# Kira7dn/Low_Level_Feature_Extraction

Hardware: AMD Instinct MI355X
Metric: images/sec, 1080p batch, full colors+shapes+shadows pipeline @1/2/4/8 MI355X (higher is better)
Workload: dtype u8

## Files before the change

low_level_feature_extraction_amd/csrc/kmeans.hip:

```cpp
#include "kmeans_common.h"

#include <mutex>
#include <type_traits>

namespace llfe {
namespace {

#ifndef LLFE_KM_CELL_MIN
#define LLFE_KM_CELL_MIN 8192
#endif
constexpr int kCellMinCubes = LLFE_KM_CELL_MIN;
#ifndef LLFE_KM_SPLIT
#define LLFE_KM_SPLIT 0
#endif
#ifndef LLFE_KM_LLOYD_QUEUE
#define LLFE_KM_LLOYD_QUEUE 0
#endif
#ifndef LLFE_KM_SUPS
#define LLFE_KM_SUPS 1
#endif
#ifndef LLFE_KM_WIDE
#define LLFE_KM_WIDE 0
#endif
#ifndef LLFE_KM_THREADS
// ... 151 lines not shown
    union {
        struct {
            unsigned long long psum[3][kParts];
            unsigned long long pD[kParts];
            unsigned long long wchunk[3][KW];
            int marg[kMaxK * kMaxK + 6 * kMaxK];
            int margc[kMaxK * kMaxK + 6 * kMaxK];
            int margs[kMaxK * kMaxK + 6 * kMaxK];
        } ppw;
        uint32_t pend[KW][kPend];
    };
    unsigned long long pex[3];
    unsigned long long S[3];
    uint32_t pbase[kParts + 1];
    uint32_t kbeg[kParts];
    uint32_t kfirst, klast;
    int pj[3];
    int icc[kMaxK][3];
    unsigned long long sel_pts;
    uint32_t stage[KW][kStage + 64];
    float thrL[3][kMaxK * kMaxK];
    int cq[KW][256];
    unsigned long long qtot;
};

static_assert(sizeof(KmSmem) * (1024 / KT) <= 160 * 1024, "KmSmem must leave room for 1024 / KT workgroups per CU");
static_assert(offsetof(KmSmem, accB) == sizeof(((KmSmem *)nullptr)->accA) &&
                  3 * KW * kSelSteps * sizeof(uint32_t) <= 2 * sizeof(((KmSmem *)nullptr)->accA),
              "selection step sums overflow the Lloyd accumulators (KT too small)");
static_assert(KW > 4 || sizeof(((KmSmem *)nullptr)->pend) <= sizeof(((KmSmem *)nullptr)->ppw),
              "pending-cube lists overflow the k-means++ state they alias");
static_assert(kPend >= 63 + 64 && (kPend & (kPend - 1)) == 0, "pending-cube list too small");

__device__ __forceinline__ Cent load_centres(const float (*c)[3]) {
    Cent r;
#pragma unroll
    for (int k = 0; k < kMaxK; k++) {
        r.x[k] = uni(c[k][0]);
        r.y[k] = uni(c[k][1]);
        r.z[k] = uni(c[k][2]);
    }
    return r;
}

__device__ __forceinline__ int moved_label(const KmSmem &sm, int i, int l) {
    for (int m = 0; m < sm.n_moved; m++)
        if (sm.moved_idx[m] == i) l = sm.moved_lbl[m];
    return l;
}

__device__ __forceinline__ int d2i(int x, int y, int z, int cx, int cy, int cz) {
    const int a = x - cx, b = y - cy, c = z - cz;
    return __mul24(a, a) + __mul24(b, b) + __mul24(c, c);
}

// ... 108 lines not shown
                      gz = (int)__builtin_rintf(az * (2.f * sc));
            p = kBisBand - ((int)__builtin_rintf(f0 * sc) + 3 * (gx + gy + gz));
            s1 = gz;
            s2 = gy - 3 * gz;
            s3 = gx - 3 * (gy + gz);
        }
        const uint32_t mlo = (uint32_t)e.mask, mhi = (uint32_t)(e.mask >> 32);
        const uint4 sg = bisector_signs(p, s1, s2, s3);
        const MaskMoments a = mask_moments(mlo & sg.x, mhi & sg.y), b = mask_moments(mlo & sg.z, mhi & sg.w);
        atomicAdd(&sm.accA[k][tid], (unsigned long long)(a.n * (uint32_t)ox + a.sx) |
                                        ((unsigned long long)(a.n * (uint32_t)oy + a.sy) << 32));
        atomicAdd(&sm.accB[k][tid], (unsigned long long)(a.n * (uint32_t)oz + a.sz) | ((unsigned long long)a.n << 32));
        atomicAdd(&sm.accA[jc][tid], (unsigned long long)(b.n * (uint32_t)ox + b.sx) |
                                         ((unsigned long long)(b.n * (uint32_t)oy + b.sy) << 32));
        atomicAdd(&sm.accB[jc][tid], (unsigned long long)(b.n * (uint32_t)oz + b.sz) | ((unsigned long long)b.n << 32));
        r.x = mlo & ~(sg.x | sg.z);
        r.y = mhi & ~(sg.y | sg.w);
        r.z = cube_origin_key(e.id);
        r.w = a.n + b.n;
    }
    return r;
}

__device__ __noinline__ uint2 gain_signs(int q, int s1, int s2, int s3) {
    uint32_t w[2] = {0u, 0u};
#pragma unroll
    for (int bit = 63; bit >= 0; bit--) {
        const int h = bit >> 5;
        w[h] = __builtin_amdgcn_alignbit(w[h], (uint32_t)q, 31);
        if (bit > 0) q += (bit & 15) == 0 ? s3 : ((bit & 3) == 0 ? s2 : s1);
    }
    return make_uint2(w[0], w[1]);
}

struct PPSplit {
    uint32_t und;
    int f[3];
    u16x2 krb;
    int ky;
};

__device__ __forceinline__ uint32_t lane_off_rel(int fill) { return (uint32_t)(__lane_id() - fill); }

constexpr int CPF = 1;
struct CubeRing {
    CubeEnt r[CPF];
    __device__ __forceinline__ void init(const CubeEnt *t, int cb, int cend, int lane) {
#pragma unroll
        for (int q = 0; q < CPF; q++) {
            r[q].mask = 0;
            r[q].id = 0;
            r[q].sums = 0;
            if (cb + q * 64 + lane < cend) r[q] = t[cb + q * 64 + lane];
        }
    }
    __device__ __forceinline__ CubeEnt next(const CubeEnt *t, int ci, int cend) {
        const CubeEnt e = r[0];
#pragma unroll
        for (int q = 0; q + 1 < CPF; q++) r[q] = r[q + 1];
        if (ci + CPF * 64 < cend) r[CPF - 1] = t[ci + CPF * 64];
        return e;
    }
// ... 46 lines not shown
        const uint32_t y = __shfl_up(x, off), hy = __shfl_up(hx, off);
        if (lane >= off) x += y, hx += hy;
    }
    const uint32_t pb = x - v, kb = hx - hv;
    sm.pbase[lane] = pb;
    sm.kbeg[lane] = kb;
    if (lane == 63) sm.pbase[kParts] = x;
    const unsigned long long ne = __ballot(v != 0);
    const int p0 = ne ? (int)__builtin_ctzll(ne) : 0, pl = ne ? 63 - (int)__builtin_clzll(ne) : 0;
    const uint32_t kf = __shfl(kb, p0), kl = __shfl(kb, pl) + __shfl(v, pl) - 1;
    if (lane == 0) {
        sm.kfirst = kf;
        sm.klast = kl;
    }
    const unsigned long long le = __ballot(pb <= idx);
    const int P = le ? 63 - (int)__builtin_clzll(le) : 0;
    return __shfl(kb, P) + (idx - __shfl(pb, P));
}

__device__ void pp_cubes(KmSmem &sm, const uint32_t *__restrict__ pts, int N, int K, uint64_t &rng,
                         const CubeEnt *__restrict__ ctab, int C, const CellEnt *__restrict__ ltab, int L,
                         const SupEnt *__restrict__ stab, int S, const uint32_t *__restrict__ part_uq, const uint32_t *__restrict__ hist,
                         const uint64_t *__restrict__ mom, unsigned long long &bytes, uint32_t &pp_pts, uint32_t &pp_sel, uint64_t &t_sel,
                         uint32_t &pp_split_cubes, uint32_t &pp_split_pts) {
    const int tid = threadIdx.x, lane = tid & 63, wid = tid >> 6;
    const uint32_t c0 = cvrng_next(rng) % (uint32_t)N;
    if (wid == 0) {
        const uint32_t a0 = key_layout(sm, part_uq, hist, c0);
        if (lane == 0) {
            const uint32_t q0 = pts[a0];
            sm.icc[0][0] = unpack_r(q0);
            sm.icc[0][1] = unpack_g(q0);
            sm.icc[0][2] = unpack_b(q0);
        }
    }
    if (tid == 0) {
        sm.fail_pts = 0;
        sm.sel_pts = 0;
    }
    if (tid >= 64 && tid < 64 + (kMaxK - 1) * 3) (&sm.icc[1][0])[tid - 64] = 0;
    unsigned long long mq[kPartMoments];
    if (wid == 1) {
#pragma unroll
        for (int q = 0; q < kPartMoments; q++) mq[q] = mom[q * kParts + lane];
    }
    __syncthreads();
    if (wid == 1) {
        const unsigned long long cx = (unsigned long long)sm.icc[0][0], cy = (unsigned long long)sm.icc[0][1],
// ... 332 lines not shown
    #pragma unroll
                for (int m = 1; m < kMaxK; m++) {
                    if (m >= KK) break;
                    Dk = k == m ? Dc[m] : Dk;
                    ky = k == m ? chg2[m] : ky;
                    krb = k == m ? chrb[m] : krb;
                }
                bool owned = true;
    #pragma unroll
                for (int m = 0; m < kMaxK; m++) {
                    if (m >= KK) break;
                    if (m != k) owned = owned & (Dc[m] - Dk - MK[m * kMaxK + k] >= 0);
                }
                const int sk = sdot(krb, ky);
                bool dec = true;
                uint32_t vv[3], und = 0u;
    #pragma unroll
                for (int j = 0; j < 3; j++) {
                    const int f = T2[j] - odot(trb[j], tg2[j]) - Dk;
                    const bool A = f - NAx[j * kMaxK + k] >= 0;
                    const bool B = f + NBx[j * kMaxK + k] <= 0;
                    dec = dec & (A | (owned & B));
                    vv[j] = A ? 0u : (uint32_t)(sdot(trb[j], tg2[j]) - sk - __mul24(n, f));
                    if (sp) {
                        sp->f[j] = f;
                        und |= (uint32_t)(owned & !A & !B) << j;
                    }
                }
                if (sp) {
                    sp->und = und;
                    sp->krb = krb;
                    sp->ky = ky;
                }
                v0 = vv[0];
                v1 = vv[1];
                v2 = vv[2];
                fail = !dec;
            };
            auto cube_vals = [&](const CubeEnt &e, uint32_t &v0, uint32_t &v1, uint32_t &v2, bool &fail,
                                 PPSplit *sp) __attribute__((always_inline)) {
                const CubeGeo g = cube_geo(e);
                box_vals(g.ox, g.oy, g.oz, g.n, g.sx, g.sy, g.sz, g.s2, Mkk, NA, NB, 3, 3, 3, v0, v1, v2, fail, sp);
            };
            auto split_owned = [&](const CubeEnt &e, const PPSplit &sp, uint32_t v0, uint32_t v1, uint32_t v2,
                                   bool &fail) __attribute__((always_inline)) {
                if (kPPSplitMin > 64) return;
                const bool so = fail && sp.und != 0u;
                const unsigned long long sb = __ballot(so);
                if (__popcll(sb) < kPPSplitMin) return;
                spl_cubes += (uint32_t)__popcll(sb);
                uint32_t und = 0u;
                if (so) {
                    und = sp.und;
                    acc0 += (und & 1u) ? 0u : v0;
                    acc1 += (und & 2u) ? 0u : v1;
                    acc2 += (und & 4u) ? 0u : v2;
                    spl_pts += e.sums & 127u;
                    fail = false;
                }
                const uint32_t mlo = (uint32_t)e.mask, mhi = (uint32_t)(e.mask >> 32);
                const uint32_t tw0 = __builtin_bit_cast(uint32_t, trb[0]), tw1 = __builtin_bit_cast(uint32_t, trb[1]),
                               tw2 = __builtin_bit_cast(uint32_t, trb[2]);
                const uint32_t kw = __builtin_bit_cast(uint32_t, sp.krb);
                while (__ballot(und != 0u)) {
                    if (und) {
                        const uint32_t m0 = 0u - (und & 1u), m1 = ~m0 & (0u - ((und >> 1) & 1u)), m2 = ~(m0 | m1);
                        und &= und - 1u;
                        const int f = (int)(((uint32_t)sp.f[0] & m0) | ((uint32_t)sp.f[1] & m1) | ((uint32_t)sp.f[2] & m2));
                        const uint32_t tw = (tw0 & m0) | (tw1 & m1) | (tw2 & m2);
                        const int tg = (int)(((uint32_t)tg2[0] & m0) | ((uint32_t)tg2[1] & m1) | ((uint32_t)tg2[2] & m2));
                        const int gx = (int)(tw >> 16) - (int)(kw >> 16), gy = tg - sp.ky,
                                  gz = (int)(tw & 0xFFFFu) - (int)(kw & 0xFFFFu);
                        const uint2 pos = gain_signs(f - 3 * (gx + gy + gz), gz, gy - 3 * gz, gx - 3 * (gy + gz));
                        const MaskMoments a = mask_moments(mlo & pos.x, mhi & pos.y);
                        const uint32_t g = (uint32_t)(__mul24(gx, (int)a.sx) + __mul24(gy, (int)a.sy) + __mul24(gz, (int)a.sz) -
                                                      __mul24((int)a.n, f));
                        acc0 += g & m0;
                        acc1 += g & m1;
                        acc2 += g & m2;
                    }
                }
            };
            auto push_cubes = [&](unsigned long long fm, const CubeEnt &e) __attribute__((always_inline)) {
                const uint32_t okey = cube_origin_key(e.id);
                const uint32_t mlo = (uint32_t)e.mask, mhi = (uint32_t)(e.mask >> 32);
                while (fm) {
    #pragma unroll
                    for (int u = 0; u < LLFE_KM_UNROLL; u++) {
                        if (u > 0 && !fm) break;
                        const int src = __builtin_ctzll(fm);
                        fm = clear_bit(fm, src);
                        const unsigned long long m =
                            ((unsigned long long)(uint32_t)__builtin_amdgcn_readlane(mhi, src) << 32) |
                            (uint32_t)__builtin_amdgcn_readlane(mlo, src);
                        const uint32_t r = __builtin_amdgcn_mbcnt_hi((uint32_t)(m >> 32),
                                                                     __builtin_amdgcn_mbcnt_lo((uint32_t)m, 0u));
                        stg[lane_sel(m, ((uint32_t)head + r) & (kStage - 1), kStage + lane)] =
                            (uint32_t)__builtin_amdgcn_readlane(okey, src) | loff;
                        head += __popcll(m);
                    }
                    while (head - tail >= 64) sum_stage(64);
                }
            };
            auto next_part = [&](int Pseg) __attribute__((always_inline)) {
// ... 35 lines not shown
                        if (cf) {
    #pragma unroll
                            for (uint32_t jj = 0; jj < 4; jj++)
                                if (jj <= nc1) ql[pre + jj] = (int)(e.first + jj);
                        }
                        __builtin_amdgcn_wave_barrier();
                        for (int b = 0; b < total; b += 64) {
                            const bool cv = b + lane < total;
                            CubeEnt ce;
                            ce.mask = 0;
                            ce.id = 0;
                            ce.sums = 0;
                            if (cv) ce = ctab[ql[b + lane]];
                            uint32_t c0 = 0, c1 = 0, c2 = 0;
                            bool cfail = false;
                            PPSplit sp;
                            sp.und = 0u;
                            if (cv) cube_vals(ce, c0, c1, c2, cfail, &sp);
                            if (cv && !cfail) {
                                acc0 += c0;
                                acc1 += c1;
                                acc2 += c2;
                            }
                            split_owned(ce, sp, c0, c1, c2, cfail);
                            const unsigned long long fm = __ballot(cv && cfail);
                            if (fm) push_cubes(fm, ce);
                        }
                        __builtin_amdgcn_wave_barrier();
                    }
                };
                int run = __builtin_amdgcn_readfirstlane(grab());
                int base = run;
                int ahead = grab();
                CellEnt en{0u, 0u, 0u, 0u};
                if (base + lane < L) en = ltab[base + lane];
                while (base < L) {
                    const bool valid = base + lane < L;
                    const CellEnt e = en;
                    int nb = base + 64;
                    if (nb >= run + kRun || nb >= L) {
                        run = __builtin_amdgcn_readfirstlane(ahead);
                        nb = run;
                        if (nb < L) ahead = grab();
                    }
                    if (nb + lane < L) en = ltab[nb + lane];
                    const int P = valid ? (int)((e.id >> 10) & 63u) : kParts;
                    uint32_t v0 = 0, v1 = 0, v2 = 0;
// ... 37 lines not shown
                    const int P = valid ? (int)((e.id >> 12) & 63u) : kParts;
                    uint32_t v0 = 0, v1 = 0, v2 = 0;
                    bool fail = false;
                    if (valid) cube_vals(e, v0, v1, v2, fail, nullptr);
                    int Pseg = __shfl(P, 0);
                    for (;;) {
                        next_part(Pseg);
                        const bool mine = P == Pseg;
                        if (mine && !fail) {
                            acc0 += v0;
                            acc1 += v1;
                            acc2 += v2;
                        }
                        const unsigned long long fm = __ballot(mine && fail);
                        if (fm) push_cubes(fm, e);
                        const unsigned long long rest = __ballot(P > Pseg && P < kParts);
                        if (!rest) break;
                        Pseg = __shfl(P, (int)__builtin_ctzll(rest));
                    }
                    base = nb;
            }
            }
            if (Pcur >= 0) {
                flush_pk();
                const unsigned long long a0 = wave_sum(acc0), a1 = wave_sum(acc1), a2 = wave_sum(acc2);
                if (lane == 0) {
                    atomicAdd(&sm.ppw.psum[0][Pcur], a0);
                    atomicAdd(&sm.ppw.psum[1][Pcur], a1);
                    atomicAdd(&sm.ppw.psum[2][Pcur], a2);
                }
            }
            if (lane == 0 && fails) atomicAdd(&sm.fail_pts, fails);
            if (spl_cubes) {
                const uint32_t np = wave_sum(spl_pts);
                if (lane == 0) {
                    atomicAdd(&sm.split_cubes, (unsigned long long)spl_cubes);
                    atomicAdd(&sm.split_pts, (unsigned long long)np);
                }
            }
        };
        switch (kk) {
            case 1: sweep(std::integral_constant<int, 1>{}); break;
            case 2: sweep(std::integral_constant<int, 2>{}); break;
            case 3: sweep(std::integral_constant<int, 3>{}); break;
            default: sweep(std::integral_constant<int, kMaxK - 1>{}); break;
        }
        __syncthreads();
        if (wid == 0) {
#pragma unroll
            for (int j = 0; j < 3; j++) {
                const unsigned long long s = wave_sum(sm.ppw.psum[j][lane]);
                if (lane == 0) sm.S[j] = sum0 - s;
            }
        }
        __syncthreads();
        int best = 0;
        double bs = 1.7976931348623157e308;
        for (int j = 0; j < 3; j++)
            if ((double)sm.S[j] < bs) {
                bs = (double)sm.S[j];
                best = j;
            }
        sum0 = sm.S[best];
        if (tid < kParts) sm.ppw.pD[tid] -= sm.ppw.psum[best][tid];
        if (tid == 0) {
            sm.icc[kk][0] = best == 0 ? tx[0] : (best == 1 ? tx[1] : tx[2]);
            sm.icc[kk][1] = best == 0 ? ty[0] : (best == 1 ? ty[1] : ty[2]);
            sm.icc[kk][2] = best == 0 ? tz[0] : (best == 1 ? tz[1] : tz[2]);
        }
    }
    __syncthreads();
    if (tid < kMaxK * 3) {
        const int k = tid / 3, j = tid % 3;
        sm.cc[k][j] = k < K ? (float)sm.icc[k][j] : kFar;
    }
    if (tid == 0) {
        bytes += 16ull * (unsigned long long)C * (unsigned long long)K + 4ull * sm.sel_pts;
        pp_pts = (uint32_t)sm.fail_pts;
        pp_sel = (uint32_t)sm.sel_pts;
        pp_split_cubes = (uint32_t)sm.split_cubes;
        pp_split_pts = (uint32_t)sm.split_pts;
        sm.fail_pts = sm.split_cubes = sm.split_pts = 0;
    }
    __syncthreads();
}

#ifndef LLFE_KM_MINW
#define LLFE_KM_MINW 4
#endif

template <bool kCubes, int kPhase, bool kQueue>
__global__ __launch_bounds__(KT, LLFE_KM_MINW) void k_kmeans(const uint32_t *__restrict__ keys, long long key_stride,
                                                   const long long *__restrict__ n_unique, int n_colors,
                                                   unsigned long long seed, ImgIndex index,
                                                   const int *__restrict__ order, int n_tasks,
                                                   int *__restrict__ queue, uint32_t *__restrict__ scratch,
                                                   long long scratch_stride, KmeansAttemptOut *__restrict__ out,
                                                   const KmeansCubes cubes) {
    static_assert(kPhase == 3 || kCubes, "the plain path runs both phases in one workgroup");
    extern __shared__ __attribute__((aligned(16))) char smem_raw[];
    KmSmem &sm = *reinterpret_cast<KmSmem *>(smem_raw);
    const int tid = threadIdx.x, lane = tid & 63, wid = tid >> 6;
    int task = (int)blockIdx.x;
    if (kQueue) {
// ... 13 lines not shown
    if (tid == 0) {
        unsigned hw, xcc;
        asm volatile("s_getreg_b32 %0, hwreg(HW_REG_HW_ID)" : "=s"(hw));
        asm volatile("s_getreg_b32 %0, hwreg(HW_REG_XCC_ID)" : "=s"(xcc));
        const uint64_t t = wall_clock64();
        if (kPhase & 1) {
            o->t_start = t;
            o->hw_id = hw;
            o->xcc_id = xcc;
        }
        if (kPhase & 2) {
            o->t_lstart = t;
            o->hw_id2 = hw;
            o->xcc_id2 = xcc;
        }
    }
    if (K <= 1) {
        if (tid == 0) {
            o->compactness = 0.0;
            o->iters = 0;
            o->bytes = 0;
            o->pp_pts = 0;
            o->pp_split_cubes = o->pp_split_pts = 0;
            o->n_cubes = 0;
            o->t_sel = 0;
            o->ll_pts = 0;
            o->split_cubes = o->split_pts = 0;
            o->split_walks = o->split_partial = 0;
            o->t_sw = 0;
            o->drift_hist = 0;
            o->pad = 0;
            o->t_end = wall_clock64();
            if (kPhase == 2) {
                o->t_start = o->t_pp = o->t_lstart;
                o->hw_id = o->hw_id2;
                o->xcc_id = o->xcc_id2;
            }
        }
        goto next_task;
    }
    const uint32_t *pts = keys + (size_t)img * key_stride;
    const int M = (N + STEP - 1) / STEP;
    const int Mw = (M + KW - 1) / KW;
    const int sb = min(M, wid * Mw), se = min(M, sb + Mw);
    const int se_full = max(sb, min(se, N / STEP));
    uint32_t *ss = scratch + ((size_t)img * kAttempts + att) * (size_t)scratch_stride;
    constexpr bool use_cubes = kCubes;
    const int C = use_cubes ? cubes.n_cubes[img] : 0;
    const CubeEnt *ctab = use_cubes ? cubes.cubes + (size_t)img * cubes.cube_stride : nullptr;
    uint32_t pp_pts = 0, pp_sel = 0, pp_split_cubes = 0, pp_split_pts = 0;
    uint64_t t_sel = 0, ll_pts = 0;
    unsigned long long bytes = use_cubes ? 0ull : 4ull * (unsigned long long)N * (unsigned long long)(K + 1);
    if (tid == 0) {
        sm.fail_pts = sm.split_cubes = sm.split_pts = 0;
        sm.split_walks = sm.split_partial = 0;
    }
#define SSLOT(slot) (ss + (size_t)(slot) * (size_t)M)

    if (kPhase & 1) {
    uint64_t rng = splitmix64(seed + (unsigned long long)index.at(img));
    if (rng == 0) rng = 0xFFFFFFFFull;
    for (int q = 0, skip = att * (1 + 6 * (K - 1)); q < skip; q++) cvrng_next(rng);

    if (use_cubes) {
        pp_cubes(sm, pts, N, K, rng, ctab, C, cubes.cells + (size_t)img * cubes.cell_stride, cubes.n_cells[img],
                 cubes.sups ? cubes.sups + (size_t)img * cubes.sup_stride : nullptr, cubes.sups ? cubes.n_sups[img] : 0,
                 cubes.part_uq + (size_t)img * kParts, cubes.part_hist ? cubes.part_hist + (size_t)img * kParts : nullptr,
                 cubes.moments + (size_t)img * kPartMoments * kParts, bytes, pp_pts, pp_sel, t_sel, pp_split_cubes, pp_split_pts);
    } else {
    int cur = 0;
    {
        const uint32_t c0 = cvrng_next(rng) % (uint32_t)N;
        const P3 q0 = unpack(pts[c0]);
        if (tid == 0) {
            sm.cc[0][0] = q0.x; sm.cc[0][1] = q0.y; sm.cc[0][2] = q0.z;
        }
        const float cx = uni(q0.x), cy = uni(q0.y), cz = uni(q0.z);
        unsigned long long wt = 0;
        for (int s = sb; s < se; s++) {
            const int i0 = s * STEP + lane * 4;
            uint32_t ls = 0;
            if (s < se_full) {
                uint4 v = *(const uint4 *)(pts + i0);
                uint32_t kq[4] = {v.x, v.y, v.z, v.w};
#pragma unroll
                for (int j = 0; j < 4; j++) {
                    P3 p = unpack(kq[j]);
                    ls += (uint32_t)d2(p.x, p.y, p.z, cx, cy, cz);
                }
            } else {
                for (int j = 0; j < 4; j++)
// ... 174 lines not shown
        sum0 = S[best];
        cur = best == 0 ? sl0 : (best == 1 ? sl1 : sl2);
        __syncthreads();
        if (tid == 0) {
            sm.cc[kk][0] = tc.x[best];
            sm.cc[kk][1] = tc.y[best];
            sm.cc[kk][2] = tc.z[best];
        }
        __syncthreads();
    }

    }
    if (tid == 0) o->t_pp = wall_clock64();
    if (tid < kMaxK * 3) (&o->pp_centers[0][0])[tid] = sm.cc[tid / 3][tid % 3];
    }
    if (kPhase == 1) {
        if (tid < kMaxK * 3) (&o->centers[0][0])[(tid / 3) * 3 + tid % 3] = sm.cc[tid / 3][tid % 3];
        if (tid == 0) {
            o->qtot = sm.qtot;
            o->bytes = bytes;
            o->pp_pts = pp_pts;
            o->pp_split_cubes = pp_split_cubes;
            o->pp_split_pts = pp_split_pts;
            o->pad = (int32_t)pp_sel;
            o->t_sel = t_sel;
        }
        goto next_task;
    }
    if (kPhase == 2) {
        if (tid < kMaxK * 3) {
            const int k = tid / 3, j = tid % 3;
            sm.cc[k][j] = k < K ? o->centers[k][j] : kFar;
        }
        if (tid == 0) sm.qtot = o->qtot;
        bytes = o->bytes;
        __syncthreads();
    }
    if (tid < kMaxK * 3) {
        int k = tid / 3, j = tid % 3;
        sm.c[k][j] = k < K ? sm.cc[k][j] : kFar;
    }
    __syncthreads();

    auto thr_tables = [&](int q) {
        const int k = q / kMaxK, j = q % kMaxK;
        const float dx = fabsf(sm.c[j][0] - sm.c[k][0]), dy = fabsf(sm.c[j][1] - sm.c[k][1]),
                    dz = fabsf(sm.c[j][2] - sm.c[k][2]);
        const bool none = j == k || j >= K || k >= K;
        sm.thrL[0][q] = none ? -__builtin_inff() : 3.f * (dx + dy + dz) + 1.f;
        sm.thrL[1][q] = none ? -__builtin_inff() : 3.f * dx + 7.f * (dy + dz) + 1.f;
        sm.thrL[2][q] = none ? -__builtin_inff() : 3.f * dx + 15.f * (dy + dz) + 1.f;
    };
    if (tid == 0) sm.next_chunk = 0;
    if (use_cubes && tid < kMaxK * kMaxK) thr_tables(tid);
#pragma unroll
    for (int k = 0; k < kMaxK; k++) {
        sm.accA[k][tid] = 0;
        sm.accB[k][tid] = 0;
    }
    __syncthreads();
    int iter = 1;
    const double eps2 = 0.2 * 0.2;
    uint64_t t_sw = 0;
    uint64_t drift_hist = 0;
    for (;;) {
        const uint64_t tsw0 = wall_clock64();
        const CentP c = pack_centres(load_centres(sm.c));
        if (use_cubes) {
            const Cent cu = load_centres(sm.c);
            f2 lw_x[3], lw_y[3], lw_z[3], lc2[3];
#pragma unroll
            for (int j = 0; j < 3; j++) {
#pragma unroll
                for (int h = 0; h < 2; h++) {
                    const int m = 2 * j + h;
                    const bool used = m < K;
                    const float cx = m < kMaxK ? cu.x[m] : 0.f, cy = m < kMaxK ? cu.y[m] : 0.f,
                                cz = m < kMaxK ? cu.z[m] : 0.f;
                    const float wx = used ? -2.f * cx : 0.f, wy = used ? -2.f * cy : 0.f, wz = used ? -2.f * cz : 0.f;
                    const float c2 = used ? cx * cx + cy * cy + cz * cz : __builtin_inff();
                    if (h == 0) {
                        lw_x[j].x = wx, lw_y[j].x = wy, lw_z[j].x = wz, lc2[j].x = c2;
                    } else {
                        lw_x[j].y = wx, lw_y[j].y = wy, lw_z[j].y = wz, lc2[j].y = c2;
                    }
                }
            }
// ... 307 lines not shown
                        unsigned long long b = (unsigned long long)(kq[jj] & 255u) | (1ull << 32);
                        atomicAdd(&sm.accA[l][tid], a);
                        atomicAdd(&sm.accB[l][tid], b);
                    }
                }
#pragma unroll
                for (int d = 0; d < PF; d++) cur[d] = nxt[d];
            }
        }
        for (int s = se_full; s < se; s++) {
            const int i0 = s * STEP + lane * 4;
            for (int jj = 0; jj < 4; jj++) {
                if (i0 + jj >= N) break;
                uint32_t kq = pts[i0 + jj];
                int l = label5p(kq, c);
                atomicAdd(&sm.accA[l][tid], (unsigned long long)((kq >> 16) & 255u) |
                                                ((unsigned long long)((kq >> 8) & 255u) << 32));
                atomicAdd(&sm.accB[l][tid], (unsigned long long)(kq & 255u) | (1ull << 32));
            }
        }
        }
        __syncthreads();
        t_sw += wall_clock64() - tsw0;
        if (tid == 0) {
            if (use_cubes) {
                bytes += 16ull * (unsigned long long)C;
                ll_pts += sm.fail_pts;
                sm.fail_pts = 0;
            } else {
                bytes += 4ull * (unsigned long long)N;
            }
        }
        for (int q = tid; q < 640; q += KT) {
            constexpr int LPP = KT / 32;
            const int v = q >> 5, part = q & 31;
            const int k = v >> 2, comp = v & 3;
            unsigned long long acc = 0;
            const unsigned long long *src = comp < 2 ? sm.accA[k] : sm.accB[k];
#pragma unroll 4
            for (int j = 0; j < LPP; j++) {
                unsigned long long wv = src[part + 32 * j];
                acc += (comp & 1) ? (wv >> 32) : (wv & 0xFFFFFFFFull);
            }
            sm.red[part][v] = acc;
        }
        __syncthreads();
#pragma unroll
        for (int k = 0; k < kMaxK; k++) {
            sm.accA[k][tid] = 0;
            sm.accB[k][tid] = 0;
        }
        for (int pass = 0;; pass++) {
            if (wid == 0) {
                const int v = lane < 20 ? lane : 0, k = v >> 2, comp = v & 3;
                unsigned long long val = 0;
                bool go = true;
                if (pass == 0) {
                    if (lane < 20) {
                        for (int part = 0; part < 32; part++) val += sm.red[part][v];
                        if (comp < 3) {
                            sm.sums[k][comp] = (long long)val;
                            sm.cprev[k][comp] = sm.c[k][comp];
                        } else {
                            sm.counts[k] = (int)val;
                        }
                    }
                    go = !__ballot(lane < 20 && comp == 3 && k < K && val == 0);
                    if (lane == 0) {
                        sm.n_moved = 0;
                        sm.flag = go ? 0 : 2;
                    }
                } else {
                    val = comp < 3 ? (unsigned long long)sm.sums[k][comp] : (unsigned long long)sm.counts[k];
                }
                if (go) {
                    const int count = (int)__shfl(val, v | 3);
                    const float scale = 1.f / (float)count;
                    const float nv = (float)(long long)val * scale;
                    const double t = (double)(nv - (comp < 3 ? sm.cprev[k][comp] : 0.f));
                    const double t2 = t * t;
                    double dist = 0.0;
                    dist += __shfl(t2, 4 * k);
                    dist += __shfl(t2, 4 * k + 1);
                    dist += __shfl(t2, 4 * k + 2);
                    if (lane < 20 && comp < 3 && k < K) sm.c[k][comp] = nv;
                    double max_shift = 0.0;
#pragma unroll
                    for (int k1 = 0; k1 < kMaxK; k1++) {
                        const double dk = __shfl(dist, 4 * k1);
                        if (k1 < K) max_shift = fmax(max_shift, dk);
                    }
                    if (use_cubes) {
                        __builtin_amdgcn_wave_barrier();
                        if (lane < kMaxK * kMaxK) thr_tables(lane);
                    }
                    if (lane == 0) {
                        sm.flag = (iter + 1 == 100 || max_shift <= eps2) ? 1 : 0;
                        sm.next_chunk = 0;
                        const int bin = (max_shift >= 0.0625) + (max_shift >= 0.25) + (max_shift >= 1.0) +
                                        (max_shift >= 4.0) + (max_shift >= 16.0) + (max_shift >= 64.0) +
                                        (max_shift >= 256.0);
                        const unsigned long long sh = 8ull * (unsigned)bin;
                        if (((drift_hist >> sh) & 255ull) < 255ull) drift_hist += 1ull << sh;
                    }
                }
            }
            __syncthreads();
            if (sm.flag != 2) break;

        for (int ek = 0; ek < K; ek++) {
            if (sm.counts[ek] != 0) continue;
            int max_k = 0;
            for (int k1 = 1; k1 < K; k1++)
                if (sm.counts[max_k] < sm.counts[k1]) max_k = k1;
            const float scale = 1.f / (float)sm.counts[max_k];
            const float bx = (float)sm.sums[max_k][0] * scale, by = (float)sm.sums[max_k][1] * scale,
                        bz = (float)sm.sums[max_k][2] * scale;
            const Cent cp = load_centres(sm.cprev);
            double md = -1.0;
            int mi = -1;
            auto visit = [&](int i) {
                P3 pp = unpack(pts[i]);
                float bd;
                int l = moved_label(sm, i, label5(pp, cp, bd));
                if (l != max_k) return;
                double d = (double)d2(pp.x, pp.y, pp.z, bx, by, bz);
// ... 44 lines not shown
                    }
                if (bi >= 0) {
                    P3 pp = unpack(pts[bi]);
                    sm.counts[max_k]--;
                    sm.counts[ek]++;
                    sm.sums[max_k][0] -= (long long)pp.x;
                    sm.sums[max_k][1] -= (long long)pp.y;
                    sm.sums[max_k][2] -= (long long)pp.z;
                    sm.sums[ek][0] += (long long)pp.x;
                    sm.sums[ek][1] += (long long)pp.y;
                    sm.sums[ek][2] += (long long)pp.z;
                    sm.moved_idx[sm.n_moved] = bi;
                    sm.moved_lbl[sm.n_moved] = ek;
                    sm.n_moved++;
                }
            }
            __syncthreads();
        }
        }
        iter++;
        if (sm.flag) break;
    }

    if (tid == 0) o->t_lloyd = wall_clock64();
    if (use_cubes) {
        if (tid == 0) {
            double acc = (double)sm.qtot;
            for (int k = 0; k < K; k++) {
                double cs = 0.0, c2 = 0.0;
                for (int j = 0; j < 3; j++) {
                    const double cj = (double)sm.c[k][j];
                    cs += cj * (double)sm.sums[k][j];
                    c2 += cj * cj;
                }
                acc -= 2.0 * cs - (double)sm.counts[k] * c2;
            }
            sm.dred[0] = acc;
            for (int w = 1; w < KW; w++) sm.dred[w] = 0.0;
        }
        __syncthreads();
    } else {
        const Cent cp = load_centres(sm.cprev);
        const Cent cn = load_centres(sm.c);
        const bool moved = sm.n_moved > 0;
        double acc = 0.0;
        for (int s = sb; s < se; s++) {
            const int i0 = s * STEP + lane * 4;
// ... 9 lines not shown
                for (int k = 1; k < kMaxK; k++) {
                    cx = l == k ? cn.x[k] : cx;
                    cy = l == k ? cn.y[k] : cy;
                    cz = l == k ? cn.z[k] : cz;
                }
                acc += (double)d2(pp.x, pp.y, pp.z, cx, cy, cz);
            }
        }
        acc = wave_sum(acc);
        if (lane == 0) sm.dred[wid] = acc;
        __syncthreads();
    }
    {
        if (tid == 0) {
            double compactness = 0.0;
            for (int w = 0; w < KW; w++) compactness += sm.dred[w];
            o->compactness = compactness;
            o->iters = iter;
            o->bytes = bytes;
            if (kPhase & 1) {
                o->pp_pts = pp_pts;
                o->pp_split_cubes = pp_split_cubes;
                o->pp_split_pts = pp_split_pts;
                o->pad = (int32_t)pp_sel;
                o->t_sel = t_sel;
            }
            o->ll_pts = ll_pts;
            o->split_cubes = sm.split_cubes;
            o->split_pts = sm.split_pts;
            o->split_walks = sm.split_walks;
            o->split_partial = sm.split_partial;
            o->t_sw = t_sw;
            o->n_cubes = (uint32_t)C;
            o->drift_hist = drift_hist;
            o->t_end = wall_clock64();
            for (int k = 0; k < kMaxK; k++) {
                for (int j = 0; j < 3; j++) o->centers[k][j] = k < K ? sm.c[k][j] : 0.f;
                o->counts[k] = k < K ? sm.counts[k] : 0;
            }
        }
    }
    }
    next_task:
    if (!kQueue) break;
    __syncthreads();
    if (tid == 0) sm.task = atomicAdd(queue, 1);
    __syncthreads();
    task = sm.task;
    __syncthreads();
    }
}


constexpr int OT = 1024;
constexpr int OMAX = 4096;
__global__ __launch_bounds__(OT) void k_kmeans_order(const long long *__restrict__ n_unique, int n,
                                                     int *__restrict__ order) {
// ... 157 lines not shown
```

low_level_feature_extraction_amd/csrc/kmeans_big.hip:

```cpp
#include "kmeans_common.h"

namespace llfe {
namespace {

using namespace km;

constexpr int BT = 512;
constexpr int BW = BT / 64;
constexpr int BSTEP = 256;

struct BigSmem {
    float c[kMaxColors][3];
    float cprev[kMaxColors][3];
    int icc[kMaxColors][3];
    long long sums[kMaxColors][3];
    int counts[kMaxColors];
    unsigned long long wacc[BW][kMaxColors][2];
    unsigned long long wtot[BW][3];
    unsigned long long scan_w[BW];
    int found_step[3];
    unsigned long long found_excl[3];
    int ci[3];
    double dred[BW];
    double maxd[BW];
// ... 395 lines not shown
        for (int qq = 0; qq < cnt; qq++) {
            int lb = l[qq];
            if (moved) lb = moved_label(sm, s * BSTEP + lane * 4 + qq, lb);
            acc += (double)d2f(fkey(kq[qq], 0), fkey(kq[qq], 1), fkey(kq[qq], 2), sm.c[lb][0], sm.c[lb][1], sm.c[lb][2]);
        }
    }
    acc = wave_sum(acc);
    if (lane == 0) sm.dred[wid] = acc;
    __syncthreads();
    if (tid == 0) {
        double compactness = 0.0;
        for (int w = 0; w < BW; w++) compactness += sm.dred[w];
        o->compactness = compactness;
        o->iters = iter;
        o->bytes = 4ull * (unsigned long long)N * (unsigned long long)(K + iter);
        o->pp_pts = 0;
        o->pp_split_cubes = o->pp_split_pts = 0;
        o->pad = 0;
        o->n_cubes = 0;
        o->t_sel = 0;
        o->ll_pts = 0;
        o->split_cubes = o->split_pts = 0;
        o->split_walks = o->split_partial = 0;
        o->t_sw = 0;
        o->drift_hist = 0;
        for (int k = 0; k < K; k++) {
            for (int j = 0; j < 3; j++) o->centers[k][j] = sm.c[k][j];
            o->counts[k] = sm.counts[k];
        }
    }
}

}

hipError_t launch_kmeans_big(const uint32_t *keys, int64_t key_stride, const int64_t *n_unique, int n, int n_colors,
                             uint64_t seed, ImgIndex index, const int32_t *order, uint32_t *scratch,
                             int64_t scratch_stride, KmeansAttemptOut *attempts, hipStream_t s) {
    if (n_colors > kMaxColors) return hipErrorInvalidValue;
    hipLaunchKernelGGL(k_kmeans_big, dim3(n * kAttempts), dim3(BT), 0, s, keys, (long long)key_stride,
                       (const long long *)n_unique, n_colors, (unsigned long long)seed, index, order,
                       scratch, (long long)scratch_stride, attempts);
    return hipGetLastError();
}

}
```

low_level_feature_extraction_amd/csrc/llfe_api.cpp:

```cpp
#include <dlfcn.h>
#include <sched.h>
#include <hip/hip_runtime.h>

#include <algorithm>
#include <chrono>
#include <atomic>
#include <cmath>
#include <condition_variable>
#include <cstdarg>
#include <cstdio>
#include <cstdlib>
#include <map>
#include <cstring>
#include <functional>
#include <mutex>
#include <string>
#include <thread>
#include <vector>

#include "../../include/llfe.h"
#include "contours.h"
#include "jpeg_huff_core.h"
#include "llfe_internal.h"

// ... 622 lines not shown
        return ctx->fail(LLFE_ERR_UNSUPPORTED, "n_colors must be in [1, LLFE_MAX_COLORS]");
    const int64_t sstride = kmeans_scratch_stride(key_stride);
    HIPCHK(ctx, W.d_order.ensure((size_t)n + 2));
    HIPCHK(ctx, W.d_kscratch.ensure((size_t)n * kAttempts * sstride));
    HIPCHK(ctx, W.d_att.ensure((size_t)n * kAttempts));
    HIPCHK(ctx, W.d_kout.ensure(n));
    W.km_n = n;
    W.km_colors = n_colors;
    ctx->km_last = &W;
    TIMED(ctx, s, "k_kmeans", 0,
          launch_kmeans(keys, key_stride, d_nuniq, n, n_colors, seed, index, W.d_order.p, W.d_kscratch.p,
                        sstride, W.d_att.p, W.d_kout.p, cubes, s));
    if (const char *path = getenv("LLFE_KM_TRACE")) {
        std::vector<KmeansAttemptOut> att((size_t)n * kAttempts);
        std::vector<int64_t> nu(n);
        HIPCHK(ctx, hipMemcpyAsync(att.data(), W.d_att.p, sizeof(KmeansAttemptOut) * att.size(),
                                   hipMemcpyDeviceToHost, s));
        HIPCHK(ctx, hipMemcpyAsync(nu.data(), d_nuniq, sizeof(int64_t) * n, hipMemcpyDeviceToHost, s));
        HIPCHK(ctx, hipStreamSynchronize(s));
        if (FILE *f = fopen(path, "a")) {
            for (int i = 0; i < n; i++)
                for (int a = 0; a < kAttempts; a++) {
                    const KmeansAttemptOut &o = att[(size_t)i * kAttempts + a];
                    fprintf(f, "%d %d %lld %d %llu %llu %u %u %llu %llu %llu %u %u %d %llu %llu %llu %llu %llu %llu %llu %u %u %u %u %u %u\n", i, a, (long long)nu[i], o.iters,
                            (unsigned long long)o.t_start, (unsigned long long)o.t_end, o.hw_id, o.xcc_id,
                            (unsigned long long)o.t_pp, (unsigned long long)o.t_lloyd, (unsigned long long)o.bytes, o.pp_pts, o.n_cubes, o.pad, (unsigned long long)o.t_sel,
                            (unsigned long long)o.ll_pts, (unsigned long long)o.t_sw, (unsigned long long)o.split_cubes,
                            (unsigned long long)o.split_pts, (unsigned long long)o.drift_hist,
                            (unsigned long long)o.t_lstart, o.hw_id2, o.xcc_id2, o.pp_split_cubes, o.pp_split_pts,
                            o.split_walks, o.split_partial);
                }
            fclose(f);
        }
    }
    return LLFE_OK;
}

bool is_light_color(int r, int g, int b) {
    const double R = r / 255.0, G = g / 255.0, B = b / 255.0;
    return 0.2126 * R + 0.7152 * G + 0.0722 * B > 0.6;
}

void fill_palette(llfe_image_result &r) {
    const int K = r.n_colors;
    int ord[kMaxColors];
    for (int i = 0; i < K; i++) ord[i] = i;
    if (K > 1) std::stable_sort(ord, ord + K, [&](int a, int b) { return r.counts[a] > r.counts[b]; });
    char hex[kMaxColors][8];
    int rgb[kMaxColors][3];
    int nh = 0;
    for (int i = 0; i < K; i++) {
        const uint8_t *c = r.centers_rgb[ord[i]];
        if ((c[0] == 255 && c[1] == 255 && c[2] == 255) || (c[0] == 0 && c[1] == 0 && c[2] == 0)) continue;
// ... 1743 lines not shown
```

low_level_feature_extraction_amd/csrc/llfe_internal.h:

```cpp
#pragma once
#include <hip/hip_runtime.h>
#include <stdint.h>

#include <vector>

#include "../../include/llfe.h"

namespace llfe {

constexpr int kTileW = 64;
constexpr int kTileH = 32;

#define LLFE_GAUSS11_F32                                                                                     \
    0x1.20c256p-7f, 0x1.bcb86ap-6f, 0x1.0ab50ap-4f, 0x1.f2464cp-4f, 0x1.6a7e1ep-3f, 0x1.9ac20ap-3f,          \
        0x1.6a7e1ep-3f, 0x1.f2464cp-4f, 0x1.0ab50ap-4f, 0x1.bcb86ap-6f, 0x1.20c256p-7f

struct StencilParams {
    float k11[11];
    uint8_t *tflag;
    const uint64_t *img_tab;
};

hipError_t launch_stencil(const uint8_t *bgr, int n, int h, int w, uint8_t *cls, uint8_t *blurred,
                          unsigned long long *shadow_sum, unsigned long long *shadow_cnt, uint2 *tile_part,
// ... 110 lines not shown
constexpr int kPartMoments = 5;

struct KmeansAttemptOut {
    double compactness;
    float centers[kMaxColors][3];
    int32_t counts[kMaxColors];
    int32_t iters;
    int32_t pad;
    uint64_t bytes;
    uint64_t t_start, t_pp, t_lloyd, t_end;
    uint32_t hw_id, xcc_id;
    uint32_t pp_pts, n_cubes;
    uint32_t pp_split_cubes, pp_split_pts;
    uint64_t t_sel;
    uint64_t ll_pts;
    uint64_t split_cubes;
    uint64_t split_pts;
    uint64_t t_sw;
    uint64_t drift_hist;
    uint64_t qtot;
    uint64_t t_lstart;
    uint32_t hw_id2, xcc_id2;
    uint32_t split_walks, split_partial;
    float pp_centers[kMaxK][3];
};

struct KmeansImageOut {
    int32_t k;
    int32_t counts[kMaxColors];
    uint8_t centers_rgb[kMaxColors][3];
    uint8_t pad[4];
    int64_t n_unique;
    double compactness;
    uint64_t bytes;
};

struct CubeEnt {
    uint64_t mask;
    uint32_t id;
    uint32_t sums;
};
static_assert(sizeof(CubeEnt) == 16, "CubeEnt is one 16-byte load");
constexpr int kMaxCubes = 1 << 18;
constexpr int kCellsPerPart = 1024;
struct CellEnt {
    uint32_t id;
// ... 104 lines not shown
```

Baseline: 37130.

## Queue split k-means++ cubes in LDS ring and drain them in full-wave walks

In k-means++ seeding, undecided owned cubes are no longer walked inline with a divergent per-lane loop over the undecided bisectors. They are appended to a per-wave LDS ring buffer that aliases the Lloyd accumulators, and the ring is drained 64 entries at a time. Each lane handles one bisector and accumulates its gain into shared per-partition sums with atomics, and any leftover bisectors are re-queued. This is meant to remove SIMD divergence. In exchange it adds LDS traffic, atomics, and a tighter shared-memory aliasing constraint. It also inlines gain_signs, moves the drift histogram and byte accounting out of the Lloyd loop, and adds walk counters to the telemetry.

```diff
diff --git a/low_level_feature_extraction_amd/csrc/kmeans.hip b/low_level_feature_extraction_amd/csrc/kmeans.hip
--- a/low_level_feature_extraction_amd/csrc/kmeans.hip
+++ b/low_level_feature_extraction_amd/csrc/kmeans.hip
@@ -197,6 +197,7 @@
     float thrL[3][kMaxK * kMaxK];
     int cq[KW][256];
     unsigned long long qtot;
+    unsigned long long drift_hist;
 };
 
 static_assert(sizeof(KmSmem) * (1024 / KT) <= 160 * 1024, "KmSmem must leave room for 1024 / KT workgroups per CU");
@@ -206,6 +207,15 @@
 static_assert(KW > 4 || sizeof(((KmSmem *)nullptr)->pend) <= sizeof(((KmSmem *)nullptr)->ppw),
               "pending-cube lists overflow the k-means++ state they alias");
 static_assert(kPend >= 63 + 64 && (kPend & (kPend - 1)) == 0, "pending-cube list too small");
+struct PPPend {
+    uint32_t list[KW][3][kPend];
+    uint32_t walks, lanes, mixed;
+};
+static_assert(sizeof(PPPend) % 4 == 0 && 3 * KW * kSelSteps * sizeof(uint32_t) + sizeof(PPPend) <= 2 * sizeof(((KmSmem *)nullptr)->accA),
+              "k-means++ pending-cube lists overlap the selection's step sums");
+__device__ __forceinline__ PPPend &pp_pend(KmSmem &sm) {
+    return *reinterpret_cast<PPPend *>(reinterpret_cast<char *>(&sm.accB[0][0]) + sizeof(sm.accB) - sizeof(PPPend));
+}
 
 __device__ __forceinline__ Cent load_centres(const float (*c)[3]) {
     Cent r;
@@ -360,7 +370,7 @@
     return r;
 }
 
-__device__ __noinline__ uint2 gain_signs(int q, int s1, int s2, int s3) {
+__device__ __forceinline__ uint2 gain_signs(int q, int s1, int s2, int s3) {
     uint32_t w[2] = {0u, 0u};
 #pragma unroll
     for (int bit = 63; bit >= 0; bit--) {
@@ -371,11 +381,46 @@
     return make_uint2(w[0], w[1]);
 }
 
+__device__ __forceinline__ uint32_t pp_walk(KmSmem &sm, int first, int n, int head, uint32_t tk0, uint32_t tk1, uint32_t tk2) {
+    const int lane = threadIdx.x & 63, wid = threadIdx.x >> 6;
+    uint32_t(*pl)[kPend] = pp_pend(sm).list[wid];
+    uint32_t rest = 0u, mlo = 0u, mhi = 0u, ent = 0u;
+    int R = -1;
+    if (lane < n) {
+        const uint32_t slot = (uint32_t)(first + lane) & (kPend - 1);
+        mlo = pl[0][slot];
+        mhi = pl[1][slot];
+        ent = pl[2][slot];
+        const int k = (int)(ent >> (kPendIdxBits + 3));
+        const uint32_t und = (ent >> kPendIdxBits) & 7u;
+        const int j = __builtin_ctz(und);
+        rest = und & (und - 1u);
+        R = (int)((ent >> 12) & 63u);
+        const int ox = R * 4, oy = (int)((ent >> 6) & 63u) * 4, oz = (int)(ent & 63u) * 4;
+        const int kx = sm.icc[k][0], ky = sm.icc[k][1], kz = sm.icc[k][2];
+        const uint32_t tk = j == 0 ? tk0 : (j == 1 ? tk1 : tk2);
+        const int tjx = (int)(tk >> 16), tjy = (int)((tk >> 8) & 255u), tjz = (int)(tk & 255u);
+        const int f = d2i(ox, oy, oz, tjx, tjy, tjz) - d2i(ox, oy, oz, kx, ky, kz);
+        const int gx = 2 * (tjx - kx), gy = 2 * (tjy - ky), gz = 2 * (tjz - kz);
+        const uint2 pos = gain_signs(f - 3 * (gx + gy + gz), gz, gy - 3 * gz, gx - 3 * (gy + gz));
+        const MaskMoments a = mask_moments(mlo & pos.x, mhi & pos.y);
+        const uint32_t g = (uint32_t)(__mul24(gx, (int)a.sx) + __mul24(gy, (int)a.sy) + __mul24(gz, (int)a.sz) - __mul24((int)a.n, f));
+        if (g) atomicAdd(&(&sm.ppw.psum[0][0])[j * kParts + R], (unsigned long long)g);
+    }
+    const unsigned long long rb = __ballot(rest != 0u);
+    if (rest) {
+        const uint32_t slot = ((uint32_t)head + __builtin_amdgcn_mbcnt_hi((uint32_t)(rb >> 32), __builtin_amdgcn_mbcnt_lo((uint32_t)rb, 0u))) & (kPend - 1);
+        pl[0][slot] = mlo;
+        pl[1][slot] = mhi;
+        pl[2][slot] = (ent & ~(7u << kPendIdxBits)) | (rest << kPendIdxBits);
+    }
+    const uint32_t mixed = __ballot(lane < n && R != __builtin_amdgcn_readfirstlane(R)) != 0ull;
+    return (uint32_t)__popcll(rb) | (mixed << 7);
+}
+
 struct PPSplit {
     uint32_t und;
-    int f[3];
-    u16x2 krb;
-    int ky;
+    int k;
 };
 
 __device__ __forceinline__ uint32_t lane_off_rel(int fill) { return (uint32_t)(__lane_id() - fill); }
@@ -468,8 +513,9 @@
                          const CubeEnt *__restrict__ ctab, int C, const CellEnt *__restrict__ ltab, int L,
                          const SupEnt *__restrict__ stab, int S, const uint32_t *__restrict__ part_uq, const uint32_t *__restrict__ hist,
                          const uint64_t *__restrict__ mom, unsigned long long &bytes, uint32_t &pp_pts, uint32_t &pp_sel, uint64_t &t_sel,
-                         uint32_t &pp_split_cubes, uint32_t &pp_split_pts) {
+                         uint32_t &pp_split_cubes, uint32_t &pp_split_pts, uint3 &pp_walks) {
     const int tid = threadIdx.x, lane = tid & 63, wid = tid >> 6;
+    if (tid == 0) pp_pend(sm).walks = pp_pend(sm).lanes = pp_pend(sm).mixed = 0u;
     const uint32_t c0 = cvrng_next(rng) % (uint32_t)N;
     if (wid == 0) {
         const uint32_t a0 = key_layout(sm, part_uq, hist, c0);
@@ -848,15 +894,11 @@
                     const bool B = f + NBx[j * kMaxK + k] <= 0;
                     dec = dec & (A | (owned & B));
                     vv[j] = A ? 0u : (uint32_t)(sdot(trb[j], tg2[j]) - sk - __mul24(n, f));
-                    if (sp) {
-                        sp->f[j] = f;
-                        und |= (uint32_t)(owned & !A & !B) << j;
-                    }
+                    if (sp) und |= (uint32_t)(owned & !A & !B) << j;
                 }
                 if (sp) {
                     sp->und = und;
-                    sp->krb = krb;
-                    sp->ky = ky;
+                    sp->k = k;
                 }
                 v0 = vv[0];
                 v1 = vv[1];
@@ -868,44 +910,41 @@
                 const CubeGeo g = cube_geo(e);
                 box_vals(g.ox, g.oy, g.oz, g.n, g.sx, g.sy, g.sz, g.s2, Mkk, NA, NB, 3, 3, 3, v0, v1, v2, fail, sp);
             };
-            auto split_owned = [&](const CubeEnt &e, const PPSplit &sp, uint32_t v0, uint32_t v1, uint32_t v2,
-                                   bool &fail) __attribute__((always_inline)) {
+            int phead = 0, ptail = 0;
+            uint32_t n_walks = 0, n_lanes = 0, n_mixed = 0;
+            const uint32_t tk0 = (uint32_t)((tx[0] << 16) | (ty[0] << 8) | tz[0]), tk1 = (uint32_t)((tx[1] << 16) | (ty[1] << 8) | tz[1]),
+                           tk2 = (uint32_t)((tx[2] << 16) | (ty[2] << 8) | tz[2]);
+            auto pp_drain = [&](int n) __attribute__((always_inline)) {
+                __builtin_amdgcn_wave_barrier();
+                const uint32_t w = (uint32_t)__builtin_amdgcn_readfirstlane((int)pp_walk(sm, ptail, n, phead, tk0, tk1, tk2));
+                __builtin_amdgcn_wave_barrier();
+                ptail += n;
+                phead += (int)(w & 127u);
+                n_walks++;
+                n_lanes += (uint32_t)n;
+                n_mixed += w >> 7;
+            };
+            auto list_owned = [&](const CubeEnt &e, const PPSplit &sp, uint32_t v0, uint32_t v1, uint32_t v2,
+                                  bool &fail) __attribute__((always_inline)) {
                 if (kPPSplitMin > 64) return;
                 const bool so = fail && sp.und != 0u;
                 const unsigned long long sb = __ballot(so);
                 if (__popcll(sb) < kPPSplitMin) return;
                 spl_cubes += (uint32_t)__popcll(sb);
-                uint32_t und = 0u;
                 if (so) {
-                    und = sp.und;
-                    acc0 += (und & 1u) ? 0u : v0;
-                    acc1 += (und & 2u) ? 0u : v1;
-                    acc2 += (und & 4u) ? 0u : v2;
+                    acc0 += (sp.und & 1u) ? 0u : v0;
+                    acc1 += (sp.und & 2u) ? 0u : v1;
+                    acc2 += (sp.und & 4u) ? 0u : v2;
                     spl_pts += e.sums & 127u;
                     fail = false;
-                }
-                const uint32_t mlo = (uint32_t)e.mask, mhi = (uint32_t)(e.mask >> 32);
-                const uint32_t tw0 = __builtin_bit_cast(uint32_t, trb[0]), tw1 = __builtin_bit_cast(uint32_t, trb[1]),
-                               tw2 = __builtin_bit_cast(uint32_t, trb[2]);
-                const uint32_t kw = __builtin_bit_cast(uint32_t, sp.krb);
-                while (__ballot(und != 0u)) {
-                    if (und) {
-                        const uint32_t m0 = 0u - (und & 1u), m1 = ~m0 & (0u - ((und >> 1) & 1u)), m2 = ~(m0 | m1);
-                        und &= und - 1u;
-                        const int f = (int)(((uint32_t)sp.f[0] & m0) | ((uint32_t)sp.f[1] & m1) | ((uint32_t)sp.f[2] & m2));
-                        const uint32_t tw = (tw0 & m0) | (tw1 & m1) | (tw2 & m2);
-                        const int tg = (int)(((uint32_t)tg2[0] & m0) | ((uint32_t)tg2[1] & m1) | ((uint32_t)tg2[2] & m2));
-                        const int gx = (int)(tw >> 16) - (int)(kw >> 16), gy = tg - sp.ky,
-                                  gz = (int)(tw & 0xFFFFu) - (int)(kw & 0xFFFFu);
-                        const uint2 pos = gain_signs(f - 3 * (gx + gy + gz), gz, gy - 3 * gz, gx - 3 * (gy + gz));
-                        const MaskMoments a = mask_moments(mlo & pos.x, mhi & pos.y);
-                        const uint32_t g = (uint32_t)(__mul24(gx, (int)a.sx) + __mul24(gy, (int)a.sy) + __mul24(gz, (int)a.sz) -
-                                                      __mul24((int)a.n, f));
-                        acc0 += g & m0;
-                        acc1 += g & m1;
-                        acc2 += g & m2;
-                    }
-                }
+                    const uint32_t slot = ((uint32_t)phead + __builtin_amdgcn_mbcnt_hi((uint32_t)(sb >> 32), __builtin_amdgcn_mbcnt_lo((uint32_t)sb, 0u))) & (kPend - 1);
+                    uint32_t(*pl)[kPend] = pp_pend(sm).list[wid];
+                    pl[0][slot] = (uint32_t)e.mask;
+                    pl[1][slot] = (uint32_t)(e.mask >> 32);
+                    pl[2][slot] = (e.id & ((1u << kPendIdxBits) - 1u)) | (sp.und << kPendIdxBits) | ((uint32_t)sp.k << (kPendIdxBits + 3));
+                }
+                phead += __popcll(sb);
+                while (phead - ptail >= 64) pp_drain(64);
             };
             auto push_cubes = [&](unsigned long long fm, const CubeEnt &e) __attribute__((always_inline)) {
                 const uint32_t okey = cube_origin_key(e.id);
@@ -987,7 +1026,7 @@
                                 acc1 += c1;
                                 acc2 += c2;
                             }
-                            split_owned(ce, sp, c0, c1, c2, cfail);
+                            list_owned(ce, sp, c0, c1, c2, cfail);
                             const unsigned long long fm = __ballot(cv && cfail);
                             if (fm) push_cubes(fm, ce);
                         }
@@ -1071,6 +1110,7 @@
             }
             }
             if (Pcur >= 0) {
+                while (phead > ptail) pp_drain(min(phead - ptail, 64));
                 flush_pk();
                 const unsigned long long a0 = wave_sum(acc0), a1 = wave_sum(acc1), a2 = wave_sum(acc2);
                 if (lane == 0) {
@@ -1085,6 +1125,9 @@
                 if (lane == 0) {
                     atomicAdd(&sm.split_cubes, (unsigned long long)spl_cubes);
                     atomicAdd(&sm.split_pts, (unsigned long long)np);
+                    atomicAdd(&pp_pend(sm).walks, n_walks);
+                    atomicAdd(&pp_pend(sm).lanes, n_lanes);
+                    atomicAdd(&pp_pend(sm).mixed, n_mixed);
                 }
             }
         };
@@ -1129,6 +1172,7 @@
         pp_sel = (uint32_t)sm.sel_pts;
         pp_split_cubes = (uint32_t)sm.split_cubes;
         pp_split_pts = (uint32_t)sm.split_pts;
+        pp_walks = make_uint3(pp_pend(sm).walks, pp_pend(sm).lanes, pp_pend(sm).mixed);
         sm.fail_pts = sm.split_cubes = sm.split_pts = 0;
     }
     __syncthreads();
@@ -1188,6 +1232,7 @@
             o->bytes = 0;
             o->pp_pts = 0;
             o->pp_split_cubes = o->pp_split_pts = 0;
+            o->pp_walks = o->pp_walk_lanes = o->pp_walk_mixed = 0;
             o->n_cubes = 0;
             o->t_sel = 0;
             o->ll_pts = 0;
@@ -1215,6 +1260,7 @@
     const int C = use_cubes ? cubes.n_cubes[img] : 0;
     const CubeEnt *ctab = use_cubes ? cubes.cubes + (size_t)img * cubes.cube_stride : nullptr;
     uint32_t pp_pts = 0, pp_sel = 0, pp_split_cubes = 0, pp_split_pts = 0;
+    uint3 pp_walks = make_uint3(0u, 0u, 0u);
     uint64_t t_sel = 0, ll_pts = 0;
     unsigned long long bytes = use_cubes ? 0ull : 4ull * (unsigned long long)N * (unsigned long long)(K + 1);
     if (tid == 0) {
@@ -1232,7 +1278,7 @@
         pp_cubes(sm, pts, N, K, rng, ctab, C, cubes.cells + (size_t)img * cubes.cell_stride, cubes.n_cells[img],
                  cubes.sups ? cubes.sups + (size_t)img * cubes.sup_stride : nullptr, cubes.sups ? cubes.n_sups[img] : 0,
                  cubes.part_uq + (size_t)img * kParts, cubes.part_hist ? cubes.part_hist + (size_t)img * kParts : nullptr,
-                 cubes.moments + (size_t)img * kPartMoments * kParts, bytes, pp_pts, pp_sel, t_sel, pp_split_cubes, pp_split_pts);
+                 cubes.moments + (size_t)img * kPartMoments * kParts, bytes, pp_pts, pp_sel, t_sel, pp_split_cubes, pp_split_pts, pp_walks);
     } else {
     int cur = 0;
     {
@@ -1453,6 +1499,9 @@
             o->pp_pts = pp_pts;
             o->pp_split_cubes = pp_split_cubes;
             o->pp_split_pts = pp_split_pts;
+            o->pp_walks = pp_walks.x;
+            o->pp_walk_lanes = pp_walks.y;
+            o->pp_walk_mixed = pp_walks.z;
             o->pad = (int32_t)pp_sel;
             o->t_sel = t_sel;
         }
@@ -1493,7 +1542,7 @@
     int iter = 1;
     const double eps2 = 0.2 * 0.2;
     uint64_t t_sw = 0;
-    uint64_t drift_hist = 0;
+    if (tid == 0) sm.drift_hist = 0;
     for (;;) {
         const uint64_t tsw0 = wall_clock64();
         const CentP c = pack_centres(load_centres(sm.c));
@@ -1847,16 +1896,9 @@
         }
         __syncthreads();
         t_sw += wall_clock64() - tsw0;
-        if (tid == 0) {
-            if (use_cubes) {
-                bytes += 16ull * (unsigned long long)C;
-                ll_pts += sm.fail_pts;
-                sm.fail_pts = 0;
-            } else {
-                bytes += 4ull * (unsigned long long)N;
-            }
-        }
-        for (int q = tid; q < 640; q += KT) {
+        int tq = tid;
+        asm volatile("" : "+v"(tq));
+        for (int q = tq; q < 640; q += KT) {
             constexpr int LPP = KT / 32;
             const int v = q >> 5, part = q & 31;
             const int k = v >> 2, comp = v & 3;
@@ -1877,11 +1919,13 @@
         }
         for (int pass = 0;; pass++) {
             if (wid == 0) {
-                const int v = lane < 20 ? lane : 0, k = v >> 2, comp = v & 3;
+                int ln = (int)__builtin_amdgcn_mbcnt_hi(~0u, __builtin_amdgcn_mbcnt_lo(~0u, 0u));
+                asm volatile("" : "+v"(ln));
+                const int v = ln < 20 ? ln : 0, k = v >> 2, comp = v & 3;
                 unsigned long long val = 0;
                 bool go = true;
                 if (pass == 0) {
-                    if (lane < 20) {
+                    if (ln < 20) {
                         for (int part = 0; part < 32; part++) val += sm.red[part][v];
                         if (comp < 3) {
                             sm.sums[k][comp] = (long long)val;
@@ -1890,8 +1934,8 @@
                             sm.counts[k] = (int)val;
                         }
                     }
-                    go = !__ballot(lane < 20 && comp == 3 && k < K && val == 0);
-                    if (lane == 0) {
+                    go = !__ballot(ln < 20 && comp == 3 && k < K && val == 0);
+                    if (ln == 0) {
                         sm.n_moved = 0;
                         sm.flag = go ? 0 : 2;
                     }
@@ -1908,7 +1952,7 @@
                     dist += __shfl(t2, 4 * k);
                     dist += __shfl(t2, 4 * k + 1);
                     dist += __shfl(t2, 4 * k + 2);
-                    if (lane < 20 && comp < 3 && k < K) sm.c[k][comp] = nv;
+                    if (ln < 20 && comp < 3 && k < K) sm.c[k][comp] = nv;
                     double max_shift = 0.0;
 #pragma unroll
                     for (int k1 = 0; k1 < kMaxK; k1++) {
@@ -1917,16 +1961,17 @@
                     }
                     if (use_cubes) {
                         __builtin_amdgcn_wave_barrier();
-                        if (lane < kMaxK * kMaxK) thr_tables(lane);
-                    }
-                    if (lane == 0) {
+                        if (ln < kMaxK * kMaxK) thr_tables(ln);
+                    }
+                    if (ln == 0) {
                         sm.flag = (iter + 1 == 100 || max_shift <= eps2) ? 1 : 0;
                         sm.next_chunk = 0;
                         const int bin = (max_shift >= 0.0625) + (max_shift >= 0.25) + (max_shift >= 1.0) +
                                         (max_shift >= 4.0) + (max_shift >= 16.0) + (max_shift >= 64.0) +
                                         (max_shift >= 256.0);
                         const unsigned long long sh = 8ull * (unsigned)bin;
-                        if (((drift_hist >> sh) & 255ull) < 255ull) drift_hist += 1ull << sh;
+                        const unsigned long long dh = sm.drift_hist;
+                        if (((dh >> sh) & 255ull) < 255ull) sm.drift_hist = dh + (1ull << sh);
                     }
                 }
             }
@@ -2017,7 +2062,11 @@
         if (sm.flag) break;
     }
 
-    if (tid == 0) o->t_lloyd = wall_clock64();
+    if (tid == 0) {
+        o->t_lloyd = wall_clock64();
+        bytes += (unsigned long long)(iter - 1) * (use_cubes ? 16ull * (unsigned long long)C : 4ull * (unsigned long long)N);
+        ll_pts = sm.fail_pts;
+    }
     if (use_cubes) {
         if (tid == 0) {
             double acc = (double)sm.qtot;
@@ -2073,6 +2122,9 @@
                 o->pp_pts = pp_pts;
                 o->pp_split_cubes = pp_split_cubes;
                 o->pp_split_pts = pp_split_pts;
+                o->pp_walks = pp_walks.x;
+                o->pp_walk_lanes = pp_walks.y;
+                o->pp_walk_mixed = pp_walks.z;
                 o->pad = (int32_t)pp_sel;
                 o->t_sel = t_sel;
             }
@@ -2083,7 +2135,7 @@
             o->split_partial = sm.split_partial;
             o->t_sw = t_sw;
             o->n_cubes = (uint32_t)C;
-            o->drift_hist = drift_hist;
+            o->drift_hist = sm.drift_hist;
             o->t_end = wall_clock64();
             for (int k = 0; k < kMaxK; k++) {
                 for (int j = 0; j < 3; j++) o->centers[k][j] = k < K ? sm.c[k][j] : 0.f;
diff --git a/low_level_feature_extraction_amd/csrc/kmeans_big.hip b/low_level_feature_extraction_amd/csrc/kmeans_big.hip
--- a/low_level_feature_extraction_amd/csrc/kmeans_big.hip
+++ b/low_level_feature_extraction_amd/csrc/kmeans_big.hip
@@ -441,6 +441,7 @@
         o->ll_pts = 0;
         o->split_cubes = o->split_pts = 0;
         o->split_walks = o->split_partial = 0;
+        o->pp_walks = o->pp_walk_lanes = o->pp_walk_mixed = 0;
         o->t_sw = 0;
         o->drift_hist = 0;
         for (int k = 0; k < K; k++) {
diff --git a/low_level_feature_extraction_amd/csrc/llfe_api.cpp b/low_level_feature_extraction_amd/csrc/llfe_api.cpp
--- a/low_level_feature_extraction_amd/csrc/llfe_api.cpp
+++ b/low_level_feature_extraction_amd/csrc/llfe_api.cpp
@@ -668,13 +668,13 @@
             for (int i = 0; i < n; i++)
                 for (int a = 0; a < kAttempts; a++) {
                     const KmeansAttemptOut &o = att[(size_t)i * kAttempts + a];
-                    fprintf(f, "%d %d %lld %d %llu %llu %u %u %llu %llu %llu %u %u %d %llu %llu %llu %llu %llu %llu %llu %u %u %u %u %u %u\n", i, a, (long long)nu[i], o.iters,
+                    fprintf(f, "%d %d %lld %d %llu %llu %u %u %llu %llu %llu %u %u %d %llu %llu %llu %llu %llu %llu %llu %u %u %u %u %u %u %u %u %u\n", i, a, (long long)nu[i], o.iters,
                             (unsigned long long)o.t_start, (unsigned long long)o.t_end, o.hw_id, o.xcc_id,
                             (unsigned long long)o.t_pp, (unsigned long long)o.t_lloyd, (unsigned long long)o.bytes, o.pp_pts, o.n_cubes, o.pad, (unsigned long long)o.t_sel,
                             (unsigned long long)o.ll_pts, (unsigned long long)o.t_sw, (unsigned long long)o.split_cubes,
                             (unsigned long long)o.split_pts, (unsigned long long)o.drift_hist,
                             (unsigned long long)o.t_lstart, o.hw_id2, o.xcc_id2, o.pp_split_cubes, o.pp_split_pts,
-                            o.split_walks, o.split_partial);
+                            o.split_walks, o.split_partial, o.pp_walks, o.pp_walk_lanes, o.pp_walk_mixed);
                 }
             fclose(f);
         }
diff --git a/low_level_feature_extraction_amd/csrc/llfe_internal.h b/low_level_feature_extraction_amd/csrc/llfe_internal.h
--- a/low_level_feature_extraction_amd/csrc/llfe_internal.h
+++ b/low_level_feature_extraction_amd/csrc/llfe_internal.h
@@ -156,6 +156,8 @@
     uint64_t t_lstart;
     uint32_t hw_id2, xcc_id2;
     uint32_t split_walks, split_partial;
+    uint32_t pp_walks, pp_walk_lanes;
+    uint32_t pp_walk_mixed;
     float pp_centers[kMaxK][3];
 };
 
```

Result: faster. 38400, median of 6 (+3.4%).
